# TXH-mercury/VALOR

Measured on AMD Instinct MI355X. Metric: pretrain samples/sec (V+A+T clip), higher is better.
Workload: dtype bf16

## Files before the change

include/valor_hip.h:

```cpp
#ifndef VALOR_HIP_H
#define VALOR_HIP_H
#include <stdint.h>
#ifdef __cplusplus
extern "C" {
#endif

#define VALOR_DT_BF16 0
#define VALOR_DT_F32 1
#define VALOR_OK 0
#define VALOR_ERR_ARG (-1)
#define VALOR_ERR_LAUNCH (-2)
#define VALOR_ACT_NONE 0
#define VALOR_ACT_GELU_ERF 1
#define VALOR_ACT_QUICK_GELU 2
#define VALOR_ACT_RELU 3
#define VALOR_ACT_TANH 4
#define VALOR_ACT_DERIV 16

int valor_gemm(void* stream, int dtype, int transA, int transB, int M, int N, int K, const void* A, int64_t lda,
               const void* B, int64_t ldb, void* C, int64_t ldc, const void* bias, int act, void* preact,
               const void* dact_aux, int64_t ldaux, float alpha, int accumulate, int out_f32, void* workspace,
               int64_t workspace_bytes, void* rowsum_out,
               int rowsum_accumulate);

// ... 5 lines not shown
    int sched_256;
    int sched_narrow;
} valor_gemm_policy;
int valor_gemm_tuned(const valor_gemm_policy* policy, void* stream, int dtype, int transA, int transB, int M, int N, int K,
                     const void* A, int64_t lda, const void* B, int64_t ldb, void* C, int64_t ldc, const void* bias, int act,
                     void* preact, const void* dact_aux, int64_t ldaux, float alpha, int accumulate, int out_f32, void* workspace,
                     int64_t workspace_bytes, void* rowsum_out, int rowsum_accumulate);
int valor_gemm_kernel_for_tuned(const valor_gemm_policy* policy, int dtype, int transA, int transB, int M, int N, int K,
                                int heavy_epilogue);

typedef struct valor_gemm_pending { unsigned char opaque[256]; } valor_gemm_pending;
int valor_gemm_deferred(void* stream, int dtype, int transA, int transB, int M, int N, int K, const void* A, int64_t lda,
                        const void* B, int64_t ldb, void* C, int64_t ldc, const void* bias, int act, void* preact,
                        const void* dact_aux, int64_t ldaux, float alpha, int accumulate, int out_f32, void* workspace,
                        int64_t workspace_bytes, void* rowsum_out, int rowsum_accumulate, valor_gemm_pending* pending);
int valor_gemm_pending_bytes(const valor_gemm_pending* pending, int64_t* bytes);
int valor_gemm_reduce_group(void* stream, int dtype, const valor_gemm_pending* pendings, int n);

int valor_gemm_set_variant(int v);
int valor_gemm_kernel_for(int dtype, int transA, int transB, int M, int N, int K, int heavy_epilogue);
int valor_gemm_set_tr_asm(int v);
int valor_gemm_set_fast_epilogue(int v);
int valor_gemm_set_policy(int key, int value);
int valor_gemm_wave128_for(int dtype, int transA, int transB, int M, int N, int K, int heavy_epilogue);
int valor_gemm_set_8ph_sched(int v);
int valor_gemm_set_narrow_sched(int v);
int valor_gemm_narrow_occupancy(void);
int valor_gemm_wide_occupancy(void);

typedef struct valor_xattn_seg {
    const void* q; const void* o; const void* dout; void* dq; const float* lse; const int* kv_range;
    int64_t q_bs, q_rs, o_bs, o_rs, do_bs, do_rs, dq_bs, dq_rs;
    int B, Sq;
    uint64_t seed, offset;
} valor_xattn_seg;
int valor_cross_attn_fwd_fused(void* stream, int dtype, const valor_xattn_seg* segs, int nseg, const void* k, const void* v, int H, int Skv,
                               int kv_bmod, int64_t k_bs, int64_t k_rs, int64_t v_bs, int64_t v_rs, float scale, float p_drop,
                               const uint64_t* rng_base);
int valor_cross_attn_bwd_fused(void* stream, int dtype, const valor_xattn_seg* segs, int nseg, const void* k, const void* v, void* dk, void* dv,
                               int H, int Skv, int kv_bmod, int64_t k_bs, int64_t k_rs, int64_t v_bs, int64_t v_rs, int64_t dk_bs,
                               int64_t dk_rs, int64_t dv_bs, int64_t dv_rs, float scale, float p_drop, const uint64_t* rng_base);

int valor_ln_part_blocks(void);
int valor_ln_set_variant(int v);
int valor_ln_set_nt(int v);
int valor_bdrln_fwd(void* stream, int dtype, const void* x, const void* bias, const void* residual, const void* gamma,
// ... 224 lines not shown
```

valor_amd/build.py:

```python
import hashlib
import os
import subprocess
import sys
from concurrent.futures import ThreadPoolExecutor

HERE = os.path.dirname(os.path.abspath(__file__))
CSRC = os.path.join(HERE, "csrc")
LIB = os.path.join(HERE, "libvalor_hip.so")
OBJDIR = os.path.join(CSRC, "_obj")
PUBLIC_HEADER = os.path.join(os.path.dirname(HERE), "include", "valor_hip.h")
HIPCC = os.environ.get("HIPCC", "/opt/rocm/bin/hipcc")
FLAGS = ["--offload-arch=gfx950", "-O3", "-std=c++17", "-fPIC", "-Wno-unused-value", "-Wno-unused-result"]


HOT_KERNELS = ("gemm_8ph_kernel", "gemm_8q_kernel", "gemm_8ph2_kernel", "gemm_glds_kernel", "gemm_splitk_reduce", "attn_res_", "attn_x_", "attn_xu_", "ln_fwd", "ln_bwd", "adamw_kernel", "xent_",
               "fine_fused_fwd", "fine_fused_fwd_fp8_kernel", "fine_ds_chunk_kernelIDF16bLi16", "win_fwd", "win_bwd_dkv", "topk_segment_kernel",
               "topk_merge_kernel", "fine_score_pairs_kernel", "grad_partial_kernel", "update_partial_kernel", "ema_kernel", "trie_constrain_kernel",
               "trie_score_level_kernel")
KNOWN_SCRATCH = ("attn_x_fwd_kernelILi8", "attn_x_bwd_kernelILi4ELb1",
                 "kernelIf")


def _sources():
    return sorted(f for f in os.listdir(CSRC) if f.endswith(".hip"))


def _headers_digest():
    h = hashlib.sha1()
    for f in sorted(os.listdir(CSRC)):
        if f.endswith(".h"):
            with open(os.path.join(CSRC, f), "rb") as fh:
                h.update(fh.read())
    with open(PUBLIC_HEADER, "rb") as fh:
        h.update(fh.read())
    return h.hexdigest()


def _compile_one(src, hdig, verbose):
    path = os.path.join(CSRC, src)
    obj = os.path.join(OBJDIR, src[:-4] + ".o")
    stamp = obj + ".sha1"
    with open(path, "rb") as fh:
        dig = hashlib.sha1(fh.read() + hdig.encode() + " ".join(FLAGS).encode()).hexdigest()
    if os.path.exists(obj) and os.path.exists(stamp) and open(stamp).read() == dig:
        return obj, False
    cmd = [HIPCC] + FLAGS + ["-Rpass-analysis=kernel-resource-usage", "-c", path, "-o", obj]
    if verbose:
        print("[valor_amd.build]", " ".join(cmd), flush=True)
    r = subprocess.run(cmd, capture_output=True, text=True)
    if r.returncode != 0:
        sys.stderr.write(r.stdout + r.stderr)
        raise RuntimeError(f"hipcc failed on {src}")
    fn = None
    bad = []
    for line in r.stderr.splitlines():
        if "Function Name:" in line:
            fn = line.split("Function Name:")[1].split()[0]
        elif "ScratchSize [bytes/lane]:" in line:
            n = int(line.split("ScratchSize [bytes/lane]:")[1].split()[0])
            if n:
                hot = any(h in fn for h in HOT_KERNELS) and not any(k in fn for k in KNOWN_SCRATCH)
                print(f"[valor_amd.build] {'ERROR' if hot else 'WARNING'}: {src}: kernel {fn} uses {n} B/lane of scratch", flush=True)
                if hot:
                    bad.append(fn)
    if bad and os.environ.get("VALOR_BUILD_STRICT", "1") != "0":
        raise RuntimeError(f"scratch in hot kernels of {src}: {bad} (see -Rpass-analysis=kernel-resource-usage; VALOR_BUILD_STRICT=0 builds anyway)")
# ... 30 lines not shown
```

valor_amd/csrc/gemm.hip:

```cpp
#include "gemm_common.h"
#include <stdlib.h>

template <typename T, bool TA, bool TB>
__global__ __launch_bounds__(256) void gemm_kernel(GemmArgs p) {
    constexpr int VEC = ElemTraits<T>::VEC;
    constexpr int BK = 8 * VEC;
    constexpr int TILE_BYTES = 128 * TILE_ROW_BYTES;
    extern __shared__ __attribute__((aligned(16))) char smem[];

    const int tid = threadIdx.x;
    const int lane = tid & 63;
    const int wave = __builtin_amdgcn_readfirstlane(tid >> 6);
    const int wm = wave >> 1, wn = wave & 1;

    const int tiles_n = (p.N + 127) >> 7;
    const int tiles_m = (p.M + 127) >> 7;
    const int logical = xcd_remap(blockIdx.x, tiles_m * tiles_n);
    const int tm = logical / tiles_n, tn = logical - tm * tiles_n;
    const int m0 = tm << 7, n0 = tn << 7;

    const int nk_total = (p.K + BK - 1) / BK;
    int ks_begin = 0, ks_end = nk_total;
    if (p.kslices > 1) {
        ks_begin = blockIdx.y * p.ksteps_per_slice;
// ... 390 lines not shown

#define VALOR_REDUCE_GROUP 8
struct ReduceGroupArgs {
    GemmArgs g[VALOR_REDUCE_GROUP];
    int first[VALOR_REDUCE_GROUP + 1];
    int n;
};
template <typename T>
__global__ __launch_bounds__(256) void gemm_splitk_reduce_group(ReduceGroupArgs a) {
    int i = 0;
    while (i + 1 < a.n && (int)blockIdx.x >= a.first[i + 1]) ++i;
    splitk_reduce_body<T>(a.g[i], blockIdx.x - a.first[i], a.first[i + 1] - a.first[i]);
}
static int reduce_blocks(const GemmArgs& p) {
    const int64_t total = (int64_t)p.M * ((p.N + 3) / 4);
    int blocks = (int)((total + 255) / 256);
    return blocks > 4096 ? 4096 : blocks;
}

static int g_gemm_variant = 4;
static inline int gemm_variant() { return GEMM_KNOB(variant, g_gemm_variant); }
extern "C" int valor_gemm_set_variant(int v) { const int o = g_gemm_variant; if (v >= 0 && v <= 4) g_gemm_variant = v; return o; }
thread_local const GemmTuning* t_gemm_tuning = nullptr;
int g_gemm_policy_default[13] = {[] { const char* e = getenv("VALOR_GEMM_NT_MINK"); return e ? atoi(e) : 768; }(),
                        [] { const char* e = getenv("VALOR_GEMM_SPLITK_BF16"); return e ? atoi(e) : 1; }(),
                        [] { const char* e = getenv("VALOR_GEMM_MIN_TILES"); return e ? atoi(e) : 256; }(),
                        [] { const char* e = getenv("VALOR_GEMM_NT_MIN_TILES"); return e ? atoi(e) : 1024; }(),
                        [] { const char* e = getenv("VALOR_GEMM_RASTER"); return e ? atoi(e) : 1000; }(),
                        [] { const char* e = getenv("VALOR_GEMM_STORE"); return e ? atoi(e) : 1000; }(),
                        [] { const char* e = getenv("VALOR_GEMM_NTA"); return e ? atoi(e) : 0; }(),
                        [] { const char* e = getenv("VALOR_GEMM_NN_MINK"); return e ? atoi(e) : 128; }(),
                        [] { const char* e = getenv("VALOR_GEMM_NARROW"); return e ? atoi(e) : 1000; }(),
                        [] { const char* e = getenv("VALOR_GEMM_MFMA32"); return e ? atoi(e) : 0; }(),
                        [] { const char* e = getenv("VALOR_GEMM_WIDE"); return e ? atoi(e) : 0; }(),
                        [] { const char* e = getenv("VALOR_GEMM_SKINNY_ALL"); return e ? atoi(e) : 0; }(),
                        [] { const char* e = getenv("VALOR_GEMM_WAVE128"); return e ? atoi(e) : 1000; }()};
extern "C" int valor_gemm_set_policy(int key, int value) {
    if (key < 0 || key > 12) return VALOR_ERR_ARG;
    const int old = g_gemm_policy_default[key];
    if (value >= 0) g_gemm_policy_default[key] = value;
    return old;
}

static bool use_8ph(int dtype, int transA, int transB, int M, int N, int K, bool heavy_epi = false) {
    if (dtype != VALOR_DT_BF16 || gemm_variant() < 3) return false;
    if ((K % 64) != 0 || K < 128 || M < 256 || N < 256) return false;
    if (gemm_variant() == 3) return true;
    const int64_t tiles256 = (int64_t)((M + 255) / 256) * ((N + 255) / 256);
    if (transA && transB) return K >= 4096;
    if (!transA && !transB) return tiles256 >= gemm_policy(2) && K >= gemm_policy(7);
    if (!transA && transB) return tiles256 >= gemm_policy(3) && K >= (heavy_epi ? 1536 : gemm_policy(0));
    return false;
}

static bool use_8ph2(int dtype, int transA, int transB, int M, int N, int K, bool heavy_epi, bool big) {
    const int mode = gemm_policy(8);
    if (dtype != VALOR_DT_BF16 || gemm_variant() != 4 || mode == 0) return false;
    if ((K % 64) != 0 || K < 128 || M < 256 || N < 128) return false;
    if (transA && !transB) return false;
    if (mode == 1) return true;
    if (mode == 2) return !big;
// ... 14 lines not shown
    return gemm_variant() == 2 ? 2 : 1;
}

static int family3_ktiles_per_workgroup(int M, int N, int K) {
    const int nk = K / 64, tiles = ((M + 255) / 256) * ((N + 255) / 256);
    int sl = 1;
    if (2 * tiles <= 256 && nk >= 24) {
        sl = 256 / tiles;
        if (sl > nk / 6) sl = nk / 6;
        if (sl > 64) sl = 64;
        if (sl < 2) sl = 1;
    }
    return (nk + sl - 1) / sl;
}
static bool use_wave128(int dtype, int transA, int transB, int M, int N, int K, bool heavy_epi) {
    const int mode = gemm_policy(12);
    if (mode == 0 || gemm_family(dtype, transA, transB, M, N, K, heavy_epi) != 3) return false;
    if (!(transA && transB)) return false;
    if (mode == 1) return true;
    return family3_ktiles_per_workgroup(M, N, K) > 48;
}
extern "C" int valor_gemm_wave128_for(int dtype, int transA, int transB, int M, int N, int K, int heavy_epilogue) {
    return use_wave128(dtype, transA, transB, M, N, K, heavy_epilogue != 0) ? 1 : 0;
}

extern "C" int valor_gemm_kernel_for(int dtype, int transA, int transB, int M, int N, int K, int heavy_epilogue) {
    return gemm_family(dtype, transA, transB, M, N, K, heavy_epilogue != 0);
}
struct TuningScope {
    const GemmTuning* prev;
    explicit TuningScope(const void* t) : prev(t_gemm_tuning) { if (t) t_gemm_tuning = (const GemmTuning*)t; }
    ~TuningScope() { t_gemm_tuning = prev; }
};
static_assert(sizeof(GemmTuning) == 17 * sizeof(int), "valor_gemm_policy layout (include/valor_hip.h)");
extern "C" int valor_gemm_kernel_for_tuned(const void* policy, int dtype, int transA, int transB, int M, int N, int K, int heavy_epilogue) {
    TuningScope scope(policy);
    return gemm_family(dtype, transA, transB, M, N, K, heavy_epilogue != 0);
}

template <int NSTAGE>
static void launch_gemm_glds(hipStream_t st, int transA, int transB, const GemmArgs& p, dim3 grid) {
    const size_t lds = NSTAGE * 32768;
#define VALOR_GLDS_LAUNCH1(TA_, TB_, F_, W_)                                                        \
    do {                                                                                            \
        static bool attr_set = false;                                                               \
        if (!attr_set) {                                                                            \
// ... 249 lines not shown
```

valor_amd/csrc/gemm8n.hip:

```cpp
#include "gemm_common.h"
#include <stdlib.h>

#if defined(N8_ABLATE) && (N8_ABLATE & 8)
#define N8_KADV(x) 0
#else
#define N8_KADV(x) (x)
#endif
#define N8_HT 16384
#define N8_OFF_B (3 * N8_HT)
#define N8_LDS (5 * N8_HT)

DEVINL bf16x8_t n8_read_frag32(const char* tile, int row, int chunk) {
    return *(const bf16x8_t*)(tile + row * TILE_ROW_BYTES + ((chunk ^ ((row >> 1) & 7)) << 4));
}
DEVINL f32x16_t n8_mma32(bf16x8_t a, bf16x8_t b, f32x16_t c) { return __builtin_amdgcn_mfma_f32_32x32x16_bf16(a, b, c, 0, 0, 0); }
DEVINL f32x4_t n8_quad(const f32x16_t& a, int q) { return (f32x4_t){a[4 * q], a[4 * q + 1], a[4 * q + 2], a[4 * q + 3]}; }

DEVINL bf16x8_t n8_read_frag_tr8(const char* img, int off, int kk) {
    const char* a = img + off + kk * (32 * 256);
    s16x4_t lo = lds_read_tr4(a), hi = lds_read_tr4(a + 4 * 256);
    return __builtin_bit_cast(bf16x8_t, __builtin_shufflevector(lo, hi, 0, 1, 2, 3, 4, 5, 6, 7));
}

template <bool TA, bool TB, bool ASMTR, bool NTS, int SCHED, bool M32>
__global__ __launch_bounds__(256, 2) void gemm_8ph2_kernel(GemmArgs p) {
    typedef bf16_t T;
    constexpr int BK = 64;
    static_assert(!M32 || (!TA && !TB), "the 32x32x16 main loop exists for k-contiguous operands");
    extern __shared__ __attribute__((aligned(16))) char smem[];
#ifdef N8_AGPR
    { float z_; asm volatile("v_accvgpr_write_b32 %0, 0" : "=a"(z_)); asm volatile("" :: "a"(z_)); }
#endif

    const int tid = threadIdx.x;
    const int lane = tid & 63;
    const int wave = __builtin_amdgcn_readfirstlane(tid >> 6);
    const int wm = wave >> 1, wn = wave & 1;
    const int fr = lane & 15, fg = lane >> 4;
    const int l31 = lane & 31, lh = lane >> 5;

    const int tiles_n = (p.N + 127) >> 7;
    const int tiles_m = (p.M + 255) >> 8;
    int logical, slice = 0;
    if (p.kslices > 1) {
        const int ntiles = tiles_m * tiles_n;
// ... 5 lines not shown
    }
    int tm = logical / tiles_n, tn = logical - tm * tiles_n;
    if (p.raster_g > 0 && p.kslices <= 1) {
        const int G = p.raster_g, per = G * tiles_m;
        const int grp = logical / per, w = logical - grp * per;
        const int gw = min(G, tiles_n - grp * G);
        tm = w / gw;
        tn = grp * G + (w - tm * gw);
    }
    const int m0 = tm << 8, n0 = tn << 7;

    const int nk_total = p.K / BK;
    int ks_begin = 0, ks_end = nk_total;
    if (p.kslices > 1) {
        ks_begin = slice * p.ksteps_per_slice;
        ks_end = ks_begin + p.ksteps_per_slice;
        if (ks_end > nk_total) ks_end = nk_total;
        if (ks_begin > nk_total) ks_begin = nk_total;
    }
    const int k_first = ks_begin * BK;
    const int ntile = ks_end - ks_begin;

#ifdef N8_STAMP
    uint64_t stamp_[5], hs_[12] = {0, 0, 0, 0, 0, 0, 0, 0, 0, 0, 0, 0};
    stamp_[0] = __builtin_amdgcn_s_memtime();
#define N8_STAMP_AT(i) stamp_[i] = __builtin_amdgcn_s_memtime()
#define N8_HSTAMP(i) do { if (rel == 5) hs_[i] = __builtin_amdgcn_s_memtime(); __builtin_amdgcn_sched_barrier(0); } while (0)
#else
#define N8_STAMP_AT(i)
#define N8_HSTAMP(i)
#endif
    f32x4_t acc[M32 ? 1 : 8][M32 ? 1 : 4];
    f32x16_t acc32[M32 ? 4 : 1][M32 ? 2 : 1];
#pragma unroll
    for (int i = 0; i < (M32 ? 1 : 8); ++i)
#pragma unroll
        for (int j = 0; j < (M32 ? 1 : 4); ++j) acc[i][j] = (f32x4_t){0.f, 0.f, 0.f, 0.f};
#pragma unroll
    for (int i = 0; i < (M32 ? 4 : 1); ++i)
#pragma unroll
        for (int j = 0; j < (M32 ? 2 : 1); ++j)
#pragma unroll
            for (int r = 0; r < 16; ++r) acc32[i][j][r] = 0.f;

    const bool do_rs = TA && p.rowsum_out != nullptr && tn == 0;
    f32x4_t racc[2][2];
#pragma unroll
    for (int i = 0; i < 2; ++i)
#pragma unroll
        for (int j = 0; j < 2; ++j) racc[i][j] = (f32x4_t){0.f, 0.f, 0.f, 0.f};
    const bf16x8_t ones = __builtin_bit_cast(bf16x8_t, (u32x4_t){0x3f803f80u, 0x3f803f80u, 0x3f803f80u, 0x3f803f80u});

    int vA[2], vB[2];
// ... 254 lines not shown
                USE_A(0);
                HALF8(1, 0, 0, fb0, RD_A(a1, 0, 1), RD_A(a1, 1, 1), RD_A(a1, 2, 1), RD_A(a1, 3, 1), , dmaB(bcur, rel + 2, 2), , dmaB(bcur, rel + 2, 3));
                ROWSUM(1, 0);
                N8_HSTAMP(6);
                LGKM_WAIT8_BARRIER();
                N8_HSTAMP(7);
                HALF8(1, 1, 0, fb1, RD_B(bnxt, 0, 0, 0, fb0, pb0), RD_B(bnxt, 0, 1, 0, fb0, pb0), , dmaA(0, a1, rel + 2, 0), dmaA(0, a1, rel + 2, 1), ,
                      dmaA(0, a1, rel + 2, 2), dmaA(0, a1, rel + 2, 3));
                N8_HSTAMP(8);
                USE_A(1);
                HALF8(1, 1, 1, fb1, RD_B(bnxt, 1, 0, 0, fb1, pb1), RD_B(bnxt, 1, 1, 0, fb1, pb1), RD_A(a2, 0, 0), RD_A(a2, 1, 0), RD_A(a2, 2, 0),
                      RD_A(a2, 3, 0), , );
                ROWSUM(1, 1);
                N8_HSTAMP(9);
                HALF8(1, 0, 1, fb0, RD_B(bnxt, 1, 0, 1, fb1, pb1), RD_B(bnxt, 1, 1, 1, fb1, pb1), , , , , , );
                N8_HSTAMP(10);
                sa0 = sa2;
            }
#undef HALF8
#undef LGKM_WAIT8_BARRIER
        }
    }
    N8_STAMP_AT(2);
    asm volatile("s_waitcnt vmcnt(0)" ::: "memory");
    __syncthreads();
    N8_STAMP_AT(3);
#ifdef N8_STAMP
    auto stamp_out = [&]() {
        asm volatile("s_waitcnt vmcnt(0)" ::: "memory");
        stamp_[4] = __builtin_amdgcn_s_memtime();
        if (lane == 0 && !TA && p.kslices <= 1) {
            uint64_t* o = (uint64_t*)p.ws + ((int64_t)blockIdx.x * 4 + wave) * 24;
            for (int i = 0; i < 5; ++i) o[i] = stamp_[i];
            for (int i = 0; i < 12; ++i) o[8 + i] = hs_[i];
            o[5] = __builtin_amdgcn_s_getreg((31 << 11) | 4);
            o[6] = __builtin_amdgcn_s_getreg((31 << 11) | 20);
        }
    };
#else
    auto stamp_out = [&]() {};
#endif
#undef RD_A
#undef RD_B
#undef USE_A
#undef USE_B
#undef MF
#undef PIN
#undef ROWSUM
#undef WAIT8_BARRIER
    if (do_rs && fg == 0) {
#pragma unroll
        for (int hh = 0; hh < 2; ++hh)
#pragma unroll
            for (int j = 0; j < 2; ++j) {
                const int m = m0 + hh * 128 + wm * 64 + (2 * wn + j) * 16 + fr;
                if (m < p.M) {
                    if (p.kslices > 1) p.rowsum_ws[(int64_t)slice * p.M + m] = racc[hh][j][0];
                    else rowsum_store<T>(p, m, racc[hh][j][0]);
                }
            }
    }

    if constexpr (!TA) if (p.fast_epi) {
        char* sB = smem;
        const int act = p.act & VALOR_ACT_MASK;
        const bool deriv = (p.act & VALOR_ACT_DERIV) != 0;
        auto write_tile = [&](bool apply_act) {
            if constexpr (M32) {
#pragma unroll
                for (int cg = 0; cg < 8; ++cg) {
                    const int col = (cg >> 2) * 64 + wn * 32 + (cg & 3) * 8 + 4 * lh;
                    const f32x4_t bias4 = load_bias4<T>(p, n0 + col);
#pragma unroll
                    for (int rg = 0; rg < 4; ++rg) {
                        const int row = (rg >> 1) * 128 + wm * 64 + (rg & 1) * 32 + l31;
                        f32x4_t v = n8_quad(acc32[rg][cg >> 2], cg & 3);
#pragma unroll
                        for (int r = 0; r < 4; ++r) v[r] = v[r] * p.alpha + bias4[r];
                        if (apply_act) {
                            float f[4] = {v[0], v[1], v[2], v[3]};
                            act_fwd_n<4>(act, f);
                            v = (f32x4_t){f[0], f[1], f[2], f[3]};
                        }
                        const u32x2_t w = {pack2_bf16(v[0], v[1]), pack2_bf16(v[2], v[3])};
                        *(u32x2_t*)(sB + row * 256 + (((col >> 3) ^ (row & 15)) << 4) + lh * 8) = w;
// ... 97 lines not shown
#pragma unroll
    for (int pass = 0; pass < 2; ++pass) {
        if (pass) __syncthreads();
        if constexpr (M32) {
#pragma unroll
            for (int mb = 0; mb < 2; ++mb)
#pragma unroll
                for (int cg = 0; cg < 8; ++cg) {
                    const int ml = wm * 64 + mb * 32 + l31;
                    const int ch = ((cg >> 2) * 16 + wn * 8 + (cg & 3) * 2 + lh) ^ (ml & 7);
                    *(f32x4_t*)(sC + ml * 128 + ch * 4) = n8_quad(acc32[pass * 2 + mb][cg >> 2], cg & 3);
                }
        } else {
#pragma unroll
            for (int mt = 0; mt < 4; ++mt)
#pragma unroll
                for (int ni = 0; ni < 4; ++ni) {
                    const int ml = wm * 64 + mt * 16 + fr;
                    const int ch = ((ni >> 1) * 16 + wn * 8 + (ni & 1) * 4 + fg) ^ (ml & 7);
                    *(f32x4_t*)(sC + ml * 128 + ch * 4) = acc[pass * 4 + mt][ni];
                }
        }
        __syncthreads();
#pragma unroll 2
        for (int it = 0; it < 8; ++it) {
            const int ml = it * 16 + (tid >> 4);
            const int c8 = tid & 15;
            const f32x4_t v0 = *(const f32x4_t*)(sC + ml * 128 + (((2 * c8) ^ (ml & 7)) << 2));
            const f32x4_t v1 = *(const f32x4_t*)(sC + ml * 128 + (((2 * c8 + 1) ^ (ml & 7)) << 2));
            const int m = m0 + pass * 128 + ml, n = n0 + c8 * 8;
            if (wsl) {
                splitk_store8(p, slice, m, n, v0, v1);
            } else {
                epilogue_store8<true, NTS ? 1 : 0>(p, m, n, v0, v1, bias0, bias1);
            }
        }
    }
    stamp_out();
}

static int g_8ph2_sched = [] { const char* e = getenv("VALOR_GEMM_N8_SCHED"); return e ? atoi(e) : 1; }();
extern "C" int valor_gemm_set_narrow_sched(int v) {
    const int old = g_8ph2_sched;
    if (v == 0 || v == 1) g_8ph2_sched = v;
    return old;
}

extern "C" int valor_gemm_set_tr_asm(int v);
extern "C" int valor_gemm_set_fast_epilogue(int v);

void launch_gemm_8ph2(hipStream_t st, int transA, int transB, const GemmArgs& p_in) {
    GemmArgs p = p_in;
    const int fast_mode = gemm_fast_epilogue_now(), tr_asm = gemm_tr_asm_now();
    const int sched_n = GEMM_KNOB(sched_narrow, g_8ph2_sched);
    const bool light_dact = p.dact_aux && (p.act & VALOR_ACT_DERIV);
    const bool plainish = fast_mode >= 2 || (!p.preact && (!p.dact_aux || light_dact));
    p.fast_epi = fast_mode && plainish && !p.out_f32 && p.kslices <= 1 && (p.N & 7) == 0 && (p.ldc & 7) == 0 && !p.rowsum_out &&
                 (!p.dact_aux || (p.ldaux & 7) == 0) && !(p.dact_aux && p.preact) && !transA && !(p.preact && (p.act & VALOR_ACT_DERIV));
    const int tiles_m = (p.M + 255) / 256, tiles_n = (p.N + 127) / 128;
    const int tiles = tiles_m * tiles_n;
    p.raster_g = 0;
    if (p.kslices <= 1 && tiles_n > 1 && gemm_policy(4) != 0) {
        if (gemm_policy(4) != 1000) {
            p.raster_g = 2 * gemm_policy(4) < tiles_n ? 2 * gemm_policy(4) : 0;
        } else {
            const double panel = 128.0 * p.K * 2.0, a_bytes = (double)p.M * p.K * 2.0, rounds = tiles / 512.0;
            const double resident = 2.5 * 1048576.0;
            const int touched = tiles_n < 64 ? tiles_n : 64;
            double best = a_bytes + (tiles_n * panel <= resident ? 8.0 * tiles_n * panel : (rounds < 1.0 ? 1.0 : rounds) * 8.0 * touched * panel);
            for (int ng = 2; ng <= tiles_n; ++ng) {
                const int G = (tiles_n + ng - 1) / ng;
                if (G * panel > resident) continue;
                const double cost = ng * a_bytes + 8.0 * tiles_n * panel;
                if (cost < 0.9 * best) { best = cost; p.raster_g = G; }
            }
        }
    }
    const bool nts = !transA && !p.out_f32 && p.kslices <= 1 && (gemm_policy(5) == 1 || (gemm_policy(5) == 1000 && p.K <= 1024));
    p.st_mode = nts ? 1 : 0;
    if (!transA && !transB && p.kslices <= 1 && !p.rowsum_out && gemm_policy(10) != 0) {
        launch_gemm_8w(st, p, tiles, nts);
        return;
    }
    dim3 grid(tiles * (p.kslices > 1 ? p.kslices : 1));
    const size_t lds = N8_LDS;
#define VALOR_8PH2_LAUNCH1(TA_, TB_, ASM_, NTS_, S_, M32_)                                                      \
    do {                                                                                                        \
        static bool attr_set = false;                                                                           \
        if (!attr_set) {                                                                                        \
            hipFuncSetAttribute((const void*)gemm_8ph2_kernel<TA_, TB_, ASM_, NTS_, S_, M32_>, hipFuncAttributeMaxDynamicSharedMemorySize, (int)lds); \
            attr_set = true;                                                                                    \
        }                                                                                                       \
        hipLaunchKernelGGL((gemm_8ph2_kernel<TA_, TB_, ASM_, NTS_, S_, M32_>), grid, dim3(256), lds, st, p);    \
    } while (0)
#define VALOR_8PH2_LAUNCH(TA_, TB_, NTS_)                                                                       \
    do {                                                                                                        \
        constexpr bool kslow_ = TA_ || TB_;                                                                     \
        if (kslow_ && !tr_asm) { VALOR_8PH2_LAUNCH1(TA_, TB_, false, NTS_, 0, false); }                         \
        else if (sched_n == 1) { VALOR_8PH2_LAUNCH1(TA_, TB_, kslow_, NTS_, 1, false); }                   \
        else { VALOR_8PH2_LAUNCH1(TA_, TB_, kslow_, NTS_, 0, false); }                                          \
    } while (0)
#define VALOR_8PH2_LAUNCH_M32(NTS_)                                                                             \
// ... 1 lines not shown
        if (sched_n == 1) { VALOR_8PH2_LAUNCH1(false, false, false, NTS_, 1, true); }                      \
        else { VALOR_8PH2_LAUNCH1(false, false, false, NTS_, 0, true); }                                        \
    } while (0)
    if (!transA && !transB && gemm_policy(9) != 0) { if (nts) VALOR_8PH2_LAUNCH_M32(true); else VALOR_8PH2_LAUNCH_M32(false); }
    else if (!transA && !transB) { if (nts) VALOR_8PH2_LAUNCH(false, false, true); else VALOR_8PH2_LAUNCH(false, false, false); }
    else if (!transA && transB) { if (nts) VALOR_8PH2_LAUNCH(false, true, true); else VALOR_8PH2_LAUNCH(false, true, false); }
    else if (transA && !transB) VALOR_8PH2_LAUNCH(true, false, false);
    else VALOR_8PH2_LAUNCH(true, true, false);
#undef VALOR_8PH2_LAUNCH_M32
#undef VALOR_8PH2_LAUNCH
#undef VALOR_8PH2_LAUNCH1
}

extern "C" int valor_gemm_narrow_occupancy(void) {
    int n = 0;
    hipFuncSetAttribute((const void*)gemm_8ph2_kernel<false, false, false, false, 0, false>, hipFuncAttributeMaxDynamicSharedMemorySize, (int)N8_LDS);
    if (hipOccupancyMaxActiveBlocksPerMultiprocessor(&n, (const void*)gemm_8ph2_kernel<false, false, false, false, 0, false>, 256, N8_LDS) != hipSuccess) return -1;
    if (gemm_policy(9) != 0) {
        int n32 = 0;
        hipFuncSetAttribute((const void*)gemm_8ph2_kernel<false, false, false, true, 1, true>, hipFuncAttributeMaxDynamicSharedMemorySize, (int)N8_LDS);
        if (hipOccupancyMaxActiveBlocksPerMultiprocessor(&n32, (const void*)gemm_8ph2_kernel<false, false, false, true, 1, true>, 256, N8_LDS) != hipSuccess) return -1;
        if (n32 < n) n = n32;
    }
    return n;
}
```

valor_amd/csrc/gemm_common.h:

```cpp
#pragma once
#include "mma.h"

struct GemmArgs {
    const void* A; const void* B; void* C;
    const void* bias;
    void* preact;
    const void* dact_aux;
    float* ws;
    int64_t lda, ldb, ldc, ldaux;
    int M, N, K;
    int act;
    int accumulate;
    int out_f32;
    int kslices;
    int ksteps_per_slice;
    float alpha;
    uint32_t bytesA, bytesB;
    void* rowsum_out;
    float* rowsum_ws;
    int rowsum_acc;
    int fast_epi;
    int raster_g;
    int st_mode;
    int ws_bf16;
// ... 125 lines not shown

template <bool FUSED = true, int NTS = -1>
DEVINL void epilogue_store8(const GemmArgs& p, int m, int n0, f32x4_t a0, f32x4_t a1, f32x4_t b0, f32x4_t b1) {
    typedef bf16_t T;
    if (m >= p.M || n0 >= p.N) return;
    const bool vec8 = n0 + 8 <= p.N && (p.ldc & 7) == 0 && !p.out_f32 && (!p.dact_aux || (p.ldaux & 7) == 0);
    if (!vec8) {
        epilogue_store<T, FUSED>(p, m, n0, a0, b0);
        epilogue_store<T, FUSED>(p, m, n0 + 4, a1, b1);
        return;
    }
    const int64_t off = (int64_t)m * p.ldc + n0;
    f32x4_t v0, v1;
#pragma unroll
    for (int r = 0; r < 4; ++r) { v0[r] = a0[r] * p.alpha + b0[r]; v1[r] = a1[r] * p.alpha + b1[r]; }
    if constexpr (FUSED) {
        const int act = p.act & VALOR_ACT_MASK;
        const bool deriv = (p.act & VALOR_ACT_DERIV) != 0;
        f32x4_t q0 = v0, q1 = v1;
        if ((act != VALOR_ACT_NONE || (deriv && p.preact)) && !p.dact_aux) {
            float f[8] = {v0[0], v0[1], v0[2], v0[3], v1[0], v1[1], v1[2], v1[3]};
            if (p.preact && deriv) {
                float g[8];
                act_fwd_deriv_n<8>(act, f, g);
                q0 = (f32x4_t){g[0], g[1], g[2], g[3]};
                q1 = (f32x4_t){g[4], g[5], g[6], g[7]};
            } else {
                act_fwd_n<8>(act, f);
            }
            v0 = (f32x4_t){f[0], f[1], f[2], f[3]};
            v1 = (f32x4_t){f[4], f[5], f[6], f[7]};
        }
        if (p.preact) {
            u32x4_t q = {pack2_bf16(q0[0], q0[1]), pack2_bf16(q0[2], q0[3]), pack2_bf16(q1[0], q1[1]), pack2_bf16(q1[2], q1[3])};
            if constexpr (NTS < 0) store_out16(p.st_mode, (T*)p.preact + off, q);
            else store_out16<NTS != 0>((T*)p.preact + off, q);
        }
        if (p.dact_aux) {
            const T* a = (const T*)p.dact_aux + (int64_t)m * p.ldaux + n0;
            const f32x4_t u0 = load4<T>(a), u1 = load4<T>(a + 4);
            if (deriv) {
                v0 *= u0; v1 *= u1;
            } else {
                float f[8] = {v0[0], v0[1], v0[2], v0[3], v1[0], v1[1], v1[2], v1[3]};
                const float x[8] = {u0[0], u0[1], u0[2], u0[3], u1[0], u1[1], u1[2], u1[3]};
                act_bwd_mul_n<8>(act, f, x);
                v0 = (f32x4_t){f[0], f[1], f[2], f[3]};
                v1 = (f32x4_t){f[4], f[5], f[6], f[7]};
            }
        }
    }
    T* c = (T*)p.C + off;
    if (p.accumulate) { v0 += load4<T>(c); v1 += load4<T>(c + 4); }
    u32x4_t o = {pack2_bf16(v0[0], v0[1]), pack2_bf16(v0[2], v0[3]), pack2_bf16(v1[0], v1[1]), pack2_bf16(v1[2], v1[3])};
    if constexpr (NTS < 0) store_out16(p.st_mode, c, o);
    else store_out16<NTS != 0>(c, o);
}

void launch_gemm_8ph(hipStream_t st, int transA, int transB, const GemmArgs& p);
void launch_gemm_8q(hipStream_t st, int transA, int transB, const GemmArgs& p);
void launch_gemm_8ph2(hipStream_t st, int transA, int transB, const GemmArgs& p);
void launch_gemm_8w(hipStream_t st, const GemmArgs& p, int tiles, bool nts);
int gemm_skinny_chunks(int K);
int launch_gemm_skinny(hipStream_t st, const GemmArgs& p);
struct GemmTuning { int key[12]; int variant, tr_asm, fast_epilogue, sched_256, sched_narrow; };
extern thread_local const GemmTuning* t_gemm_tuning;
extern int g_gemm_policy_default[13];
static inline int gemm_policy(int k) {
    const GemmTuning* o = t_gemm_tuning;
    return (o && k < 12 && o->key[k] >= 0) ? o->key[k] : g_gemm_policy_default[k];
}
#define GEMM_KNOB(FIELD_, GLOBAL_) ((t_gemm_tuning && t_gemm_tuning->FIELD_ >= 0) ? t_gemm_tuning->FIELD_ : (GLOBAL_))
int gemm_tr_asm_now();
int gemm_fast_epilogue_now();
```

valor_amd/lib.py:

```python
import ctypes
import os

_HERE = os.path.dirname(os.path.abspath(__file__))
LIB_PATH = os.environ.get("VALOR_HIP_LIB") or os.path.join(_HERE, "libvalor_hip.so")

DT_BF16 = 0
DT_F32 = 1

ACT_NONE, ACT_GELU_ERF, ACT_QUICK_GELU, ACT_RELU, ACT_TANH = 0, 1, 2, 3, 4
ACT_DERIV = 16

_c = ctypes
_vp, _i, _i64, _u64, _f = _c.c_void_p, _c.c_int, _c.c_int64, _c.c_uint64, _c.c_float

class GemmPolicy(_c.Structure):
    _fields_ = [("key", _i * 12), ("variant", _i), ("tr_asm", _i), ("fast_epilogue", _i), ("sched_256", _i), ("sched_narrow", _i)]
    KEYS = dict(nt_min_k=0, splitk_bf16=1, min_tiles=2, nt_min_tiles=3, raster=4, store=5, nta=6, nn_min_k=7, narrow=8, mfma32=9, wide=10, skinny=11)

    @classmethod
    def make(cls, **kw):
        p = cls()
        for i in range(12):
            p.key[i] = -1
        p.variant = p.tr_asm = p.fast_epilogue = p.sched_256 = p.sched_narrow = -1
# ... 19 lines not shown

class CapevalTables(_c.Structure):
    POINTERS = RewardTables.POINTERS + ("ref_sym_ptr", "ref_syms")
    _fields_ = [(k, _vp) for k in POINTERS] + [("ref_len", _c.c_double), ("n_global", _c.c_int32), ("n_clips", _c.c_int32)]


class CapevalSummary(_c.Structure):
    _fields_ = [("value", _c.c_double * 6), ("total", _c.c_int64 * 10)]


SIGNATURES = {
    "valor_gemm": [_vp, _i, _i, _i, _i, _i, _i, _vp, _i64, _vp, _i64, _vp, _i64, _vp, _i, _vp, _vp, _i64,
                   _f, _i, _i, _vp, _i64, _vp, _i],
    "valor_gemm_tuned": [_vp, _vp, _i, _i, _i, _i, _i, _i, _vp, _i64, _vp, _i64, _vp, _i64, _vp, _i, _vp, _vp, _i64,
                         _f, _i, _i, _vp, _i64, _vp, _i],
    "valor_gemm_kernel_for_tuned": [_vp, _i, _i, _i, _i, _i, _i, _i],
    "valor_gemm_deferred": [_vp, _i, _i, _i, _i, _i, _i, _vp, _i64, _vp, _i64, _vp, _i64, _vp, _i, _vp, _vp, _i64,
                            _f, _i, _i, _vp, _i64, _vp, _i, _vp],
    "valor_gemm_pending_bytes": [_vp, _vp],
    "valor_gemm_reduce_group": [_vp, _i, _vp, _i],
    "valor_gemm_set_variant": [_i],
    "valor_gemm_kernel_for": [_i, _i, _i, _i, _i, _i, _i],
    "valor_gemm_wave128_for": [_i, _i, _i, _i, _i, _i, _i],
    "valor_gemm_set_tr_asm": [_i],
    "valor_gemm_set_fast_epilogue": [_i],
    "valor_gemm_set_policy": [_i, _i],
    "valor_gemm_set_8ph_sched": [_i],
    "valor_gemm_set_narrow_sched": [_i],
    "valor_gemm_narrow_occupancy": [],
    "valor_gemm_wide_occupancy": [],
    "valor_ln_part_blocks": [],
    "valor_ln_set_variant": [_i],
    "valor_ln_set_nt": [_i],
    "valor_bdrln_fwd": [_vp, _i, _vp, _vp, _vp, _vp, _vp, _vp, _vp, _vp, _vp, _i64, _i, _f, _f, _u64, _u64, _vp, _i64, _vp],
    "valor_bdrln_bwd": [_vp, _i, _vp, _vp, _vp, _vp, _vp, _vp, _vp, _vp, _vp, _vp, _vp, _i64, _i, _f, _u64, _u64, _vp, _i64, _vp],
    "valor_patchify3d": [_vp, _i, _vp, _vp, _i, _i, _i, _i, _i, _i],
    "valor_group_mean_fwd": [_vp, _i, _vp, _vp, _i64, _i, _i],
    "valor_group_mean_bwd": [_vp, _i, _vp, _vp, _i64, _i, _i],
    "valor_win_attn_workspace_floats": [_i, _i, _i, _i],
    "valor_win_attn_set_variant": [_i],
    "valor_win_attn_fwd": [_vp, _i, _vp, _vp, _vp, _vp, _vp, _vp, _vp, _i, _i, _i, _i, _i, _i, _i, _f],
    "valor_win_attn_bwd": [_vp, _i, _vp, _vp, _vp, _vp, _vp, _vp, _vp, _vp, _vp, _vp, _vp, _vp, _i, _vp, _i64, _i, _i, _i, _i, _i, _i, _i, _f],
    "valor_colsum_finalize": [_vp, _i, _vp, _i, _i, _vp, _i, _i],
    "valor_colsum_finalize3": [_vp, _i, _vp, _vp, _i, _vp, _vp, _i, _vp, _vp, _i, _i, _i],
    "valor_attn_set_variant": [_i],
    "valor_attn_set_res_pipeline": [_i],
# ... 117 lines not shown
```

Baseline: 581.0.

## Add two-output LDS-staged epilogue variant of narrow GEMM for activation+derivative outputs

Builds a specialised copy of the narrow 8ph2 GEMM kernel whose epilogue computes the activation and its derivative together. Both bf16 tiles are staged through LDS and written with coalesced 16-byte stores, and the second half's math is interleaved with the first half's stores. Bias is prefetched into registers before the main loop. It targets the cost of writing both C and preact in the forward MLP GEMMs, at the price of extra registers and LDS barriers, a separate kernel instantiation, and a policy gate (default mode restricts it to K<=1024).

Result: no change. 585.1 (median of 6 runs) (+0.7%).

```diff
diff --git a/include/valor_hip.h b/include/valor_hip.h
--- a/include/valor_hip.h
+++ b/include/valor_hip.h
@@ -51,6 +51,7 @@
 int valor_gemm_set_tr_asm(int v);
 int valor_gemm_set_fast_epilogue(int v);
 int valor_gemm_set_policy(int key, int value);
+int valor_gemm_epi2_for(int dtype, int transA, int transB, int M, int N, int K, int act);
 int valor_gemm_wave128_for(int dtype, int transA, int transB, int M, int N, int K, int heavy_epilogue);
 int valor_gemm_set_8ph_sched(int v);
 int valor_gemm_set_narrow_sched(int v);
diff --git a/valor_amd/build.py b/valor_amd/build.py
--- a/valor_amd/build.py
+++ b/valor_amd/build.py
@@ -1,5 +1,6 @@
 import hashlib
 import os
+import re
 import subprocess
 import sys
 from concurrent.futures import ThreadPoolExecutor
@@ -13,7 +14,7 @@
 FLAGS = ["--offload-arch=gfx950", "-O3", "-std=c++17", "-fPIC", "-Wno-unused-value", "-Wno-unused-result"]
 
 
-HOT_KERNELS = ("gemm_8ph_kernel", "gemm_8q_kernel", "gemm_8ph2_kernel", "gemm_glds_kernel", "gemm_splitk_reduce", "attn_res_", "attn_x_", "attn_xu_", "ln_fwd", "ln_bwd", "adamw_kernel", "xent_",
+HOT_KERNELS = ("gemm_8ph_kernel", "gemm_8q_kernel", "gemm_8ph2_kernel", "gemm_8ph2e_kernel", "gemm_glds_kernel", "gemm_splitk_reduce", "attn_res_", "attn_x_", "attn_xu_", "ln_fwd", "ln_bwd", "adamw_kernel", "xent_",
                "fine_fused_fwd", "fine_fused_fwd_fp8_kernel", "fine_ds_chunk_kernelIDF16bLi16", "win_fwd", "win_bwd_dkv", "topk_segment_kernel",
                "topk_merge_kernel", "fine_score_pairs_kernel", "grad_partial_kernel", "update_partial_kernel", "ema_kernel", "trie_constrain_kernel",
                "trie_score_level_kernel")
@@ -41,7 +42,11 @@
     obj = os.path.join(OBJDIR, src[:-4] + ".o")
     stamp = obj + ".sha1"
     with open(path, "rb") as fh:
-        dig = hashlib.sha1(fh.read() + hdig.encode() + " ".join(FLAGS).encode()).hexdigest()
+        text = fh.read()
+    for inc in re.findall(rb'^#include "([^"]+\.hip)"', text, re.M):
+        with open(os.path.join(CSRC, inc.decode()), "rb") as fh:
+            text += fh.read()
+    dig = hashlib.sha1(text + hdig.encode() + " ".join(FLAGS).encode()).hexdigest()
     if os.path.exists(obj) and os.path.exists(stamp) and open(stamp).read() == dig:
         return obj, False
     cmd = [HIPCC] + FLAGS + ["-Rpass-analysis=kernel-resource-usage", "-c", path, "-o", obj]
diff --git a/valor_amd/csrc/gemm.hip b/valor_amd/csrc/gemm.hip
--- a/valor_amd/csrc/gemm.hip
+++ b/valor_amd/csrc/gemm.hip
@@ -436,7 +436,7 @@
 static inline int gemm_variant() { return GEMM_KNOB(variant, g_gemm_variant); }
 extern "C" int valor_gemm_set_variant(int v) { const int o = g_gemm_variant; if (v >= 0 && v <= 4) g_gemm_variant = v; return o; }
 thread_local const GemmTuning* t_gemm_tuning = nullptr;
-int g_gemm_policy_default[13] = {[] { const char* e = getenv("VALOR_GEMM_NT_MINK"); return e ? atoi(e) : 768; }(),
+int g_gemm_policy_default[14] = {[] { const char* e = getenv("VALOR_GEMM_NT_MINK"); return e ? atoi(e) : 768; }(),
                         [] { const char* e = getenv("VALOR_GEMM_SPLITK_BF16"); return e ? atoi(e) : 1; }(),
                         [] { const char* e = getenv("VALOR_GEMM_MIN_TILES"); return e ? atoi(e) : 256; }(),
                         [] { const char* e = getenv("VALOR_GEMM_NT_MIN_TILES"); return e ? atoi(e) : 1024; }(),
@@ -448,9 +448,10 @@
                         [] { const char* e = getenv("VALOR_GEMM_MFMA32"); return e ? atoi(e) : 0; }(),
                         [] { const char* e = getenv("VALOR_GEMM_WIDE"); return e ? atoi(e) : 0; }(),
                         [] { const char* e = getenv("VALOR_GEMM_SKINNY_ALL"); return e ? atoi(e) : 0; }(),
-                        [] { const char* e = getenv("VALOR_GEMM_WAVE128"); return e ? atoi(e) : 1000; }()};
+                        [] { const char* e = getenv("VALOR_GEMM_WAVE128"); return e ? atoi(e) : 1000; }(),
+                        [] { const char* e = getenv("VALOR_GEMM_EPI2"); return e ? atoi(e) : 1000; }()};
 extern "C" int valor_gemm_set_policy(int key, int value) {
-    if (key < 0 || key > 12) return VALOR_ERR_ARG;
+    if (key < 0 || key > 13) return VALOR_ERR_ARG;
     const int old = g_gemm_policy_default[key];
     if (value >= 0) g_gemm_policy_default[key] = value;
     return old;
@@ -511,6 +512,23 @@
 }
 extern "C" int valor_gemm_wave128_for(int dtype, int transA, int transB, int M, int N, int K, int heavy_epilogue) {
     return use_wave128(dtype, transA, transB, M, N, K, heavy_epilogue != 0) ? 1 : 0;
+}
+
+extern "C" int valor_gemm_set_narrow_sched(int v);
+bool gemm_use_epi2(int dtype, int transA, int transB, int M, int N, int K, int act) {
+    const int mode = gemm_policy(13);
+    if (mode == 0 || transA || transB || !(act & VALOR_ACT_DERIV)) return false;
+    const int a = act & VALOR_ACT_MASK;
+    if (a != VALOR_ACT_GELU_ERF && a != VALOR_ACT_QUICK_GELU && a != VALOR_ACT_RELU) return false;
+    if (gemm_family(dtype, transA, transB, M, N, K, false) != 4 || (N & 7) != 0) return false;
+    if (gemm_policy(9) != 0 || gemm_policy(10) != 0 || GEMM_KNOB(sched_narrow, valor_gemm_set_narrow_sched(-1)) != 1) return false;
+    const int tiles = ((M + 255) / 256) * ((N + 127) / 128), nk = K / 64;
+    if (2 * tiles <= 512 && nk >= 24) return false;
+    if (mode == 1) return true;
+    return K <= 1024;
+}
+extern "C" int valor_gemm_epi2_for(int dtype, int transA, int transB, int M, int N, int K, int act) {
+    return gemm_use_epi2(dtype, transA, transB, M, N, K, act) ? 1 : 0;
 }
 
 extern "C" int valor_gemm_kernel_for(int dtype, int transA, int transB, int M, int N, int K, int heavy_epilogue) {
diff --git a/valor_amd/csrc/gemm8n.hip b/valor_amd/csrc/gemm8n.hip
--- a/valor_amd/csrc/gemm8n.hip
+++ b/valor_amd/csrc/gemm8n.hip
@@ -21,6 +21,101 @@
     s16x4_t lo = lds_read_tr4(a), hi = lds_read_tr4(a + 4 * 256);
     return __builtin_bit_cast(bf16x8_t, __builtin_shufflevector(lo, hi, 0, 1, 2, 3, 4, 5, 6, 7));
 }
+
+#ifdef N8_EPI2
+#ifdef N8_STAMP
+#define N8_ES_PARAM , uint64_t* es_
+#define N8_ES_ARG , es_
+#define N8_ESTAMP(i) do { es_[i] = __builtin_amdgcn_s_memtime(); __builtin_amdgcn_sched_barrier(0); } while (0)
+#else
+#define N8_ES_PARAM
+#define N8_ES_ARG
+#define N8_ESTAMP(i)
+#endif
+template <int ACT, bool NTS>
+DEVINL void n8_epi2_tile(const GemmArgs& p, char* smem, const f32x4_t (&acc)[8][4], const f32x4_t (&bias)[4], int m0, int n0, int tid, int wm,
+                         int wn, int fr, int fg N8_ES_PARAM) {
+    typedef bf16_t T;
+    char* const imY = smem;
+    char* const imG = smem + 32768;
+    auto woff = [&](int mt, int ni) {
+        const int chunk = (ni >> 1) * 8 + wn * 4 + (ni & 1) * 2 + (fg >> 1);
+        return (wm * 64 + mt * 16 + fr) * 256 + ((chunk ^ fr) << 4) + (fg & 1) * 8;
+    };
+    auto eval = [&](int mh, int q, u32x2_t& wy, u32x2_t& wg) {
+        const f32x4_t a = acc[mh * 4 + (q >> 2)][q & 3], b = bias[q & 3];
+        float f[4], g[4];
+#pragma unroll
+        for (int r = 0; r < 4; ++r) f[r] = a[r] * p.alpha + b[r];
+#pragma unroll
+        for (int r = 0; r < 4; ++r) act_fwd_deriv_c<ACT>(f[r], f[r], g[r]);
+        wy = (u32x2_t){pack2_bf16(f[0], f[1]), pack2_bf16(f[2], f[3])};
+        wg = (u32x2_t){pack2_bf16(g[0], g[1]), pack2_bf16(g[2], g[3])};
+    };
+    const int rrow = tid >> 4, rc = tid & 15;
+    const int roff = rrow * 256 + ((rc ^ rrow) << 4);
+    const int n = n0 + rc * 8;
+    auto store2 = [&](int mh, int it, u32x4_t vy, u32x4_t vg) {
+        const int m = m0 + mh * 128 + it * 16 + rrow;
+        if (m < p.M && n < p.N) {
+            const int64_t off = (int64_t)m * p.ldc + n;
+            store_out16<NTS>((T*)p.C + off, vy);
+            store_out16<NTS>((T*)p.preact + off, vg);
+        }
+    };
+#define N8_LDS_BARRIER()                                                                                          \
+    do {                                                                                                          \
+        __builtin_amdgcn_sched_barrier(0);                                                                        \
+        asm volatile("s_waitcnt lgkmcnt(0)" ::: "memory");                                                        \
+        __builtin_amdgcn_s_barrier();                                                                             \
+        __builtin_amdgcn_sched_barrier(0);                                                                        \
+    } while (0)
+#pragma unroll
+    for (int q = 0; q < 16; ++q) {
+        u32x2_t wy, wg;
+        eval(0, q, wy, wg);
+        *(u32x2_t*)(imY + woff(q >> 2, q & 3)) = wy;
+        *(u32x2_t*)(imG + woff(q >> 2, q & 3)) = wg;
+    }
+    N8_LDS_BARRIER();
+    N8_ESTAMP(0);
+    u32x2_t hy[16], hg[16];
+    u32x4_t cy = *(const u32x4_t*)(imY + roff), cg = *(const u32x4_t*)(imG + roff);
+#pragma unroll
+    for (int it = 0; it < 8; ++it) {
+        u32x4_t ny = cy, ng = cg;
+        if (it < 7) {
+            ny = *(const u32x4_t*)(imY + roff + (it + 1) * 4096);
+            ng = *(const u32x4_t*)(imG + roff + (it + 1) * 4096);
+        }
+        store2(0, it, cy, cg);
+        eval(1, 2 * it, hy[2 * it], hg[2 * it]);
+        eval(1, 2 * it + 1, hy[2 * it + 1], hg[2 * it + 1]);
+        asm volatile("" : "+v"(hy[2 * it][0]), "+v"(hy[2 * it][1]), "+v"(hg[2 * it][0]), "+v"(hg[2 * it][1]), "+v"(hy[2 * it + 1][0]),
+                     "+v"(hy[2 * it + 1][1]), "+v"(hg[2 * it + 1][0]), "+v"(hg[2 * it + 1][1]));
+        cy = ny; cg = ng;
+        __builtin_amdgcn_sched_barrier(0);
+    }
+    N8_ESTAMP(1);
+    N8_LDS_BARRIER();
+#pragma unroll
+    for (int q = 0; q < 16; ++q) {
+        *(u32x2_t*)(imY + woff(q >> 2, q & 3)) = hy[q];
+        *(u32x2_t*)(imG + woff(q >> 2, q & 3)) = hg[q];
+    }
+    N8_LDS_BARRIER();
+    N8_ESTAMP(2);
+    u32x4_t ry[8], rg[8];
+#pragma unroll
+    for (int it = 0; it < 8; ++it) {
+        ry[it] = *(const u32x4_t*)(imY + roff + it * 4096);
+        rg[it] = *(const u32x4_t*)(imG + roff + it * 4096);
+    }
+#pragma unroll
+    for (int it = 0; it < 8; ++it) store2(1, it, ry[it], rg[it]);
+#undef N8_LDS_BARRIER
+}
+#endif
 
 template <bool TA, bool TB, bool ASMTR, bool NTS, int SCHED, bool M32>
 __global__ __launch_bounds__(256, 2) void gemm_8ph2_kernel(GemmArgs p) {
@@ -72,13 +167,23 @@
     const int ntile = ks_end - ks_begin;
 
 #ifdef N8_STAMP
-    uint64_t stamp_[5], hs_[12] = {0, 0, 0, 0, 0, 0, 0, 0, 0, 0, 0, 0};
+    uint64_t stamp_[5], hs_[12] = {0, 0, 0, 0, 0, 0, 0, 0, 0, 0, 0, 0}, es_[4] = {0, 0, 0, 0};
     stamp_[0] = __builtin_amdgcn_s_memtime();
 #define N8_STAMP_AT(i) stamp_[i] = __builtin_amdgcn_s_memtime()
 #define N8_HSTAMP(i) do { if (rel == 5) hs_[i] = __builtin_amdgcn_s_memtime(); __builtin_amdgcn_sched_barrier(0); } while (0)
 #else
 #define N8_STAMP_AT(i)
 #define N8_HSTAMP(i)
+#endif
+#ifdef N8_EPI2
+    uint32_t braw[4][4];
+#pragma unroll
+    for (int ni = 0; ni < 4; ++ni) {
+        const int col = n0 + (ni >> 1) * 64 + wn * 32 + (ni & 1) * 16 + 4 * fg;
+        const uint16_t* bp = (p.bias && col < p.N) ? (const uint16_t*)p.bias + col : (const uint16_t*)p.A;
+#pragma unroll
+        for (int r = 0; r < 4; ++r) braw[ni][r] = bp[r];
+    }
 #endif
     f32x4_t acc[M32 ? 1 : 8][M32 ? 1 : 4];
     f32x16_t acc32[M32 ? 4 : 1][M32 ? 2 : 1];
@@ -379,6 +484,19 @@
         }
     }
     N8_STAMP_AT(2);
+#ifdef N8_EPI2
+    static_assert(!TA && !TB && !M32, "the two-output tile epilogue is built for the k-contiguous 16 x 16 main loop");
+    f32x4_t ebias[4];
+#pragma unroll
+    for (int ni = 0; ni < 4; ++ni) {
+        const bool has = p.bias && n0 + (ni >> 1) * 64 + wn * 32 + (ni & 1) * 16 + 4 * fg < p.N;
+#pragma unroll
+        for (int r = 0; r < 4; ++r) {
+            asm volatile("" : "+v"(braw[ni][r]));
+            ebias[ni][r] = has ? bf16_bits_to_f32(braw[ni][r]) : 0.f;
+        }
+    }
+#endif
     asm volatile("s_waitcnt vmcnt(0)" ::: "memory");
     __syncthreads();
     N8_STAMP_AT(3);
@@ -390,6 +508,7 @@
             uint64_t* o = (uint64_t*)p.ws + ((int64_t)blockIdx.x * 4 + wave) * 24;
             for (int i = 0; i < 5; ++i) o[i] = stamp_[i];
             for (int i = 0; i < 12; ++i) o[8 + i] = hs_[i];
+            for (int i = 0; i < 4; ++i) o[20 + i] = es_[i];
             o[5] = __builtin_amdgcn_s_getreg((31 << 11) | 4);
             o[6] = __builtin_amdgcn_s_getreg((31 << 11) | 20);
         }
@@ -418,6 +537,15 @@
             }
     }
 
+#ifdef N8_EPI2
+    switch (p.act & VALOR_ACT_MASK) {
+        case VALOR_ACT_GELU_ERF: n8_epi2_tile<VALOR_ACT_GELU_ERF, NTS>(p, smem, acc, ebias, m0, n0, tid, wm, wn, fr, fg N8_ES_ARG); break;
+        case VALOR_ACT_QUICK_GELU: n8_epi2_tile<VALOR_ACT_QUICK_GELU, NTS>(p, smem, acc, ebias, m0, n0, tid, wm, wn, fr, fg N8_ES_ARG); break;
+        default: n8_epi2_tile<VALOR_ACT_RELU, NTS>(p, smem, acc, ebias, m0, n0, tid, wm, wn, fr, fg N8_ES_ARG); break;
+    }
+    stamp_out();
+    return;
+#endif
     if constexpr (!TA) if (p.fast_epi) {
         char* sB = smem;
         const int act = p.act & VALOR_ACT_MASK;
@@ -561,6 +689,9 @@
                 }
         }
         __syncthreads();
+#ifdef N8_STAMP
+        es_[pass * 2] = __builtin_amdgcn_s_memtime();
+#endif
 #pragma unroll 2
         for (int it = 0; it < 8; ++it) {
             const int ml = it * 16 + (tid >> 4);
@@ -574,10 +705,14 @@
                 epilogue_store8<true, NTS ? 1 : 0>(p, m, n, v0, v1, bias0, bias1);
             }
         }
+#ifdef N8_STAMP
+        if (pass == 0) es_[1] = __builtin_amdgcn_s_memtime();
+#endif
     }
     stamp_out();
 }
 
+#ifndef N8_EPI2
 static int g_8ph2_sched = [] { const char* e = getenv("VALOR_GEMM_N8_SCHED"); return e ? atoi(e) : 1; }();
 extern "C" int valor_gemm_set_narrow_sched(int v) {
     const int old = g_8ph2_sched;
@@ -617,6 +752,11 @@
     }
     const bool nts = !transA && !p.out_f32 && p.kslices <= 1 && (gemm_policy(5) == 1 || (gemm_policy(5) == 1000 && p.K <= 1024));
     p.st_mode = nts ? 1 : 0;
+    if (p.preact && !p.dact_aux && !p.accumulate && !p.out_f32 && p.kslices <= 1 && !p.rowsum_out && (p.ldc & 7) == 0 && sched_n == 1 &&
+        gemm_use_epi2(VALOR_DT_BF16, transA, transB, p.M, p.N, p.K, p.act)) {
+        launch_gemm_8ph2_epi2(st, p, tiles, nts);
+        return;
+    }
     if (!transA && !transB && p.kslices <= 1 && !p.rowsum_out && gemm_policy(10) != 0) {
         launch_gemm_8w(st, p, tiles, nts);
         return;
@@ -664,5 +804,8 @@
         if (hipOccupancyMaxActiveBlocksPerMultiprocessor(&n32, (const void*)gemm_8ph2_kernel<false, false, false, true, 1, true>, 256, N8_LDS) != hipSuccess) return -1;
         if (n32 < n) n = n32;
     }
+    const int ne = gemm_8ph2_epi2_occupancy();
+    if (ne < n) n = ne;
     return n;
 }
+#endif
diff --git a/valor_amd/csrc/gemm8n_epi2.hip b/valor_amd/csrc/gemm8n_epi2.hip
--- /dev/null
+++ b/valor_amd/csrc/gemm8n_epi2.hip
@@ -0,0 +1,28 @@
+#define N8_EPI2 1
+#define gemm_8ph2_kernel gemm_8ph2e_kernel
+#include "gemm8n.hip"
+#undef gemm_8ph2_kernel
+
+void launch_gemm_8ph2_epi2(hipStream_t st, const GemmArgs& p, int tiles, bool nts) {
+#define VALOR_EPI2_LAUNCH(NTS_)                                                                                  \
+    do {                                                                                                         \
+        static bool attr_set = false;                                                                            \
+        if (!attr_set) {                                                                                         \
+            hipFuncSetAttribute((const void*)gemm_8ph2e_kernel<false, false, false, NTS_, 1, false>, hipFuncAttributeMaxDynamicSharedMemorySize, (int)N8_LDS); \
+            attr_set = true;                                                                                     \
+        }                                                                                                        \
+        hipLaunchKernelGGL((gemm_8ph2e_kernel<false, false, false, NTS_, 1, false>), dim3(tiles), dim3(256), N8_LDS, st, p); \
+    } while (0)
+    if (nts) VALOR_EPI2_LAUNCH(true);
+    else VALOR_EPI2_LAUNCH(false);
+#undef VALOR_EPI2_LAUNCH
+}
+
+int gemm_8ph2_epi2_occupancy() {
+    int n = 0, m = 0;
+    hipFuncSetAttribute((const void*)gemm_8ph2e_kernel<false, false, false, false, 1, false>, hipFuncAttributeMaxDynamicSharedMemorySize, (int)N8_LDS);
+    hipFuncSetAttribute((const void*)gemm_8ph2e_kernel<false, false, false, true, 1, false>, hipFuncAttributeMaxDynamicSharedMemorySize, (int)N8_LDS);
+    if (hipOccupancyMaxActiveBlocksPerMultiprocessor(&n, (const void*)gemm_8ph2e_kernel<false, false, false, false, 1, false>, 256, N8_LDS) != hipSuccess) return -1;
+    if (hipOccupancyMaxActiveBlocksPerMultiprocessor(&m, (const void*)gemm_8ph2e_kernel<false, false, false, true, 1, false>, 256, N8_LDS) != hipSuccess) return -1;
+    return m < n ? m : n;
+}
diff --git a/valor_amd/csrc/gemm_common.h b/valor_amd/csrc/gemm_common.h
--- a/valor_amd/csrc/gemm_common.h
+++ b/valor_amd/csrc/gemm_common.h
@@ -171,7 +171,11 @@
             float f[8] = {v0[0], v0[1], v0[2], v0[3], v1[0], v1[1], v1[2], v1[3]};
             if (p.preact && deriv) {
                 float g[8];
+#if defined(N8_EPI_ABLATE) && (N8_EPI_ABLATE & 1)
+                for (int r = 0; r < 8; ++r) g[r] = f[r];
+#else
                 act_fwd_deriv_n<8>(act, f, g);
+#endif
                 q0 = (f32x4_t){g[0], g[1], g[2], g[3]};
                 q1 = (f32x4_t){g[4], g[5], g[6], g[7]};
             } else {
@@ -182,8 +186,12 @@
         }
         if (p.preact) {
             u32x4_t q = {pack2_bf16(q0[0], q0[1]), pack2_bf16(q0[2], q0[3]), pack2_bf16(q1[0], q1[1]), pack2_bf16(q1[2], q1[3])};
+#if defined(N8_EPI_ABLATE) && (N8_EPI_ABLATE & 6)
+            asm volatile("" :: "v"(q));
+#else
             if constexpr (NTS < 0) store_out16(p.st_mode, (T*)p.preact + off, q);
             else store_out16<NTS != 0>((T*)p.preact + off, q);
+#endif
         }
         if (p.dact_aux) {
             const T* a = (const T*)p.dact_aux + (int64_t)m * p.ldaux + n0;
@@ -202,19 +210,26 @@
     T* c = (T*)p.C + off;
     if (p.accumulate) { v0 += load4<T>(c); v1 += load4<T>(c + 4); }
     u32x4_t o = {pack2_bf16(v0[0], v0[1]), pack2_bf16(v0[2], v0[3]), pack2_bf16(v1[0], v1[1]), pack2_bf16(v1[2], v1[3])};
+#if defined(N8_EPI_ABLATE) && (N8_EPI_ABLATE & 4)
+    asm volatile("" :: "v"(o));
+#else
     if constexpr (NTS < 0) store_out16(p.st_mode, c, o);
     else store_out16<NTS != 0>(c, o);
+#endif
 }
 
 void launch_gemm_8ph(hipStream_t st, int transA, int transB, const GemmArgs& p);
 void launch_gemm_8q(hipStream_t st, int transA, int transB, const GemmArgs& p);
 void launch_gemm_8ph2(hipStream_t st, int transA, int transB, const GemmArgs& p);
 void launch_gemm_8w(hipStream_t st, const GemmArgs& p, int tiles, bool nts);
+bool gemm_use_epi2(int dtype, int transA, int transB, int M, int N, int K, int act);
+void launch_gemm_8ph2_epi2(hipStream_t st, const GemmArgs& p, int tiles, bool nts);
+int gemm_8ph2_epi2_occupancy();
 int gemm_skinny_chunks(int K);
 int launch_gemm_skinny(hipStream_t st, const GemmArgs& p);
 struct GemmTuning { int key[12]; int variant, tr_asm, fast_epilogue, sched_256, sched_narrow; };
 extern thread_local const GemmTuning* t_gemm_tuning;
-extern int g_gemm_policy_default[13];
+extern int g_gemm_policy_default[14];
 static inline int gemm_policy(int k) {
     const GemmTuning* o = t_gemm_tuning;
     return (o && k < 12 && o->key[k] >= 0) ? o->key[k] : g_gemm_policy_default[k];
diff --git a/valor_amd/lib.py b/valor_amd/lib.py
--- a/valor_amd/lib.py
+++ b/valor_amd/lib.py
@@ -65,6 +65,7 @@
     "valor_gemm_set_variant": [_i],
     "valor_gemm_kernel_for": [_i, _i, _i, _i, _i, _i, _i],
     "valor_gemm_wave128_for": [_i, _i, _i, _i, _i, _i, _i],
+    "valor_gemm_epi2_for": [_i, _i, _i, _i, _i, _i, _i],
     "valor_gemm_set_tr_asm": [_i],
     "valor_gemm_set_fast_epilogue": [_i],
     "valor_gemm_set_policy": [_i, _i],
```
